# archinetai/audio-diffusion-pytorch

Hardware: NVIDIA H100
Metric: audio-seconds/sec (2ch, 2^18 len) VSampler 50-step (higher is better)
Workload: dtype bf16

## Files before the change

audio_diffusion_pytorch_b200/csrc/common.cuh:

```cuda
#pragma once
#include <cuda.h>
#include <cuda_runtime.h>
#include <stdarg.h>
#include <stdint.h>
#include <stdio.h>

#include "../../include/adp_b200.h"

namespace adp {

int set_error(const char* fmt, ...);

#define ADP_CHECK(cond, ...)                         \
  do {                                               \
    if (!(cond)) return ::adp::set_error(__VA_ARGS__); \
  } while (0)

#define ADP_CUDA(expr)                                                                   \
  do {                                                                                   \
    cudaError_t e_ = (expr);                                                             \
    if (e_ != cudaSuccess)                                                               \
      return ::adp::set_error("%s failed: %s (%s:%d)", #expr, cudaGetErrorString(e_),    \
                              __FILE__, __LINE__);                                       \
  } while (0)

#define ADP_LAUNCH_CHECK() ADP_CUDA(cudaGetLastError())

int make_tmap_bf16(CUtensorMap* out, const void* base, int rank, const uint64_t* dims,
                   const uint64_t* strides_bytes, const uint32_t* box, int swizzle_bytes);

inline cudaStream_t as_stream(adp_stream_t s) { return reinterpret_cast<cudaStream_t>(s); }

struct SmemAttrCache { size_t set[64] = {}; };
template <typename Kern>
inline cudaError_t ensure_dyn_smem(Kern kernel, size_t bytes, SmemAttrCache& cache) {
  int dev = 0;
  cudaError_t e = cudaGetDevice(&dev);
  if (e != cudaSuccess) return e;
  size_t& cur = cache.set[dev & 63];
  if (bytes <= cur) return cudaSuccess;
  e = cudaFuncSetAttribute((const void*)kernel, cudaFuncAttributeMaxDynamicSharedMemorySize, (int)bytes);
  if (e == cudaSuccess) cur = bytes;
  return e;
}

extern int g_pdl;
template <typename Kern, typename... Args>
inline cudaError_t launch_k(Kern kernel, dim3 grid, dim3 block, size_t smem, cudaStream_t st,
                            Args... args) {
  cudaLaunchConfig_t cfg = {};
  cfg.gridDim = grid;
  cfg.blockDim = block;
  cfg.dynamicSmemBytes = smem;
  cfg.stream = st;
  cudaLaunchAttribute attr[1];
  attr[0].id = cudaLaunchAttributeProgrammaticStreamSerialization;
  attr[0].val.programmaticStreamSerializationAllowed = g_pdl ? 1 : 0;
  cfg.attrs = attr;
  cfg.numAttrs = 1;
  void* ptrs[] = {(void*)&args...};
  return cudaLaunchKernelExC(&cfg, (const void*)kernel, ptrs);
}

int num_sms();

template <typename K>
inline int one_wave_gx(K kernel, int threads, size_t smem, int B, int n_tiles) {
  int occ = 1;
  if (cudaOccupancyMaxActiveBlocksPerMultiprocessor(&occ, kernel, threads, smem) != cudaSuccess || occ < 1)
    occ = 1;
  int gx = (occ * num_sms()) / B;
  if (gx < 1) gx = 1;
  if (gx > n_tiles) gx = n_tiles;
  return gx;
}

inline int blocks_per_batch(int n_tiles, int B, int z = 1) {
  int gx = (num_sms() * 4 + B * z - 1) / (B * z);
  if (gx > n_tiles) gx = n_tiles;
  return gx < 1 ? 1 : gx;
}

inline bool ln_row_layout(int C, int* lpr, int* vpl) {
  const int vpr = C / 8;
  if (vpr <= 32) {
    int p = 1;
    while (p < vpr) p <<= 1;
    *lpr = p; *vpl = 1;
  } else {
    *lpr = 32; *vpl = (vpr + 31) / 32;
  }
  return *lpr * *vpl != vpr;
}

inline int capped_grid(int64_t n, int threads) {
  int64_t g = (n + threads - 1) / threads;
  if (g < 1) g = 1;
  if (g > num_sms() * 16) g = num_sms() * 16;
  return static_cast<int>(g);
}

}
```

audio_diffusion_pytorch_b200/csrc/conv_gemm.cu:

```cuda
#include "common.cuh"
#include "ptx.cuh"

namespace adp {

int g_debug[8] = {0, 0, 0, 0, 0, 0, 0, 0};

constexpr int kMaxStages = 8;
constexpr int kMaxGroups = 8;
constexpr int kSmemPerSM = 228 * 1024;
constexpr int kSmemPerBlock = 227 * 1024;

struct Gemm2Params {
  __nv_bfloat16* out;
  const __nv_bfloat16* residual;
  const float* bias;
  const float* gate;
  double* stats;
  int B, T, tiles_per_batch, c_in, ldo;
  int n_pad, n_valid;
  int ntaps, tap_off0, up_factor;
  int groups, group_size, group_shift;
  int out_fp32, ld_gate;
  int n_tiles_n, total_tiles, tiles_per_cta;
  int a_rows;
// ... 11 lines not shown

struct TileInfo {
  int b, t0, n0, phase, ch0, ntaps, min_off;
};

template <int BM>
__device__ __forceinline__ TileInfo tile_info(const Gemm2Params& p, int tile, int BN) {
  TileInfo ti;
  const int m_tile = tile / p.n_tiles_n;
  const int n_tile = tile - m_tile * p.n_tiles_n;
  ti.b = m_tile / p.tiles_per_batch;
  ti.t0 = (m_tile - ti.b * p.tiles_per_batch) * BM;
  ti.n0 = n_tile * BN;
  ti.phase = ti.n0 / p.n_pad;
  ti.ch0 = ti.n0 - ti.phase * p.n_pad;
  if (p.up_factor > 1) {
    if (ti.phase == 0) { ti.ntaps = 2; ti.min_off = -1; }
    else if (ti.phase == p.up_factor - 1) { ti.ntaps = 2; ti.min_off = 0; }
    else { ti.ntaps = 1; ti.min_off = 0; }
  } else {
    ti.ntaps = p.ntaps;
    ti.min_off = p.tap_off0;
  }
  return ti;
}

__device__ __forceinline__ float silu_tanh(float z) {
  float t;
  asm("tanh.approx.f32 %0, %1;" : "=f"(t) : "f"(0.5f * z));
  const float hz = 0.5f * z;
  return fmaf(hz, t, hz);
}

struct WarpStats {
  int cur_g = -1;
  float s = 0.f, q = 0.f;
  template <int NW>
  __device__ __forceinline__ void flush(float (*slots)[NW], int w, int lane) {
    const float ws = warp_sum(s), wq = warp_sum(q);
    if (lane == 0 && cur_g >= 0) { slots[2 * cur_g][w] += ws; slots[2 * cur_g + 1][w] += wq; }
    s = 0.f; q = 0.f;
  }
  template <int NW>
  __device__ __forceinline__ void add(float v, int g, float (*slots)[NW], int w, int lane) {
    if (g != cur_g) { flush(slots, w, lane); cur_g = g; }
    s += v; q += v * v;
  }
};

struct NarrowStats {
  int ch0 = -1;
  float s[4] = {0.f, 0.f, 0.f, 0.f}, q[4] = {0.f, 0.f, 0.f, 0.f};
  __device__ __forceinline__ void add(int k, float v) { s[k] += v; q[k] += v * v; }
  template <int NW>
  __device__ __forceinline__ void flush(float (*slots)[NW], int w, int lane, int shift, int groups) {
    if (ch0 >= 0) {
#pragma unroll
      for (int k = 0; k < 4; ++k) {
        float a = s[k], b = q[k];
#pragma unroll
        for (int o = 4; o < 32; o <<= 1) {
          a += __shfl_xor_sync(0xffffffffu, a, o);
          b += __shfl_xor_sync(0xffffffffu, b, o);
        }
        if (shift == 2) {
          a += __shfl_xor_sync(0xffffffffu, a, 1);
          b += __shfl_xor_sync(0xffffffffu, b, 1);
        }
        const int col = shift == 0 ? ch0 + 2 * lane + k : ch0 + 8 * k + 2 * (lane & 3);
        const int g = col >> shift;
        if (lane < 4 && (shift != 2 || !(lane & 1)) && (shift != 0 || k < 2) && g < groups) {
          slots[2 * g][w] += a;
          slots[2 * g + 1][w] += b;
        }
        s[k] = 0.f; q[k] = 0.f;
      }
    }
    ch0 = -1;
  }
};

template <int BM> constexpr int gemm_threads() { return 2 * BM + 32; }

template <int BM, int BN, int SW, bool XF, bool NARROW>
__global__ void __launch_bounds__(gemm_threads<BM>(), BM == 256 ? 1 : (BN <= 32 ? 3 : (BN <= 64 ? 2 : 1)))
conv_gemm2_kernel(const __grid_constant__ CUtensorMap tmA, const __grid_constant__ CUtensorMap tmW,
                  const Gemm2Params p) {
  static_assert(!NARROW || (BN <= 64 && !XF), "narrow statistics registers: BN <= 64 without XF");
  static_assert(BM == 128 || (BM == 256 && BN == 64 && !XF && !NARROW),
                "256-row tiles: BN = 64, without the A transform or the narrow statistics");
  constexpr int BK = SW / 2;
  constexpr int NACC = BN / 2;
  constexpr int kConsumers = 2 * BM;
  constexpr int kConsumerWarps = BM / 16;
  constexpr uint32_t kWTapBytes = BN * SW;
  extern __shared__ uint8_t smem_raw[];
  __shared__ uint64_t full_bar[kMaxStages], empty_bar[kMaxStages];
  __shared__ float s_part[2 * kMaxGroups][kConsumerWarps];
  __shared__ __align__(16) float s_coef[XF ? 2 * 1024 : 4];

  pdl_launch_dependents();
  const int warp = warp_id_uniform();
  const int lane = threadIdx.x & 31;
  const uint32_t raw = smem_u32(smem_raw);
  uint8_t* ring = smem_raw + ((1024u - (raw & 1023u)) & 1023u);

  const int tile_begin = blockIdx.x * p.tiles_per_cta;
  int tile_end = tile_begin + p.tiles_per_cta;
  if (tile_end > p.total_tiles) tile_end = p.total_tiles;

  if (threadIdx.x < 2 * kMaxGroups * kConsumerWarps) (&s_part[0][0])[threadIdx.x] = 0.f;
  if (warp == kConsumerWarps && lane == 0) {
    for (int s = 0; s < p.n_stages; ++s) { mbar_init(&full_bar[s], 1); mbar_init(&empty_bar[s], kConsumerWarps); }
    fence_mbar_init();
    tma_prefetch_desc(&tmA);
    tma_prefetch_desc(&tmW);
  }
  __syncthreads();
  if (warp == kConsumerWarps) {
    const uint32_t a_bytes = static_cast<uint32_t>(BM / 128) * p.a_rows * SW;
    const int total_it = (tile_end - tile_begin) * p.k_stages;
    int early = 0;
    if (p.early_w) {
      early = total_it < p.n_stages ? total_it : p.n_stages;
      if (elect_one()) {
        int tile = tile_begin, ks = 0;
        for (int it = 0; it < early; ++it) {
          const TileInfo ti = tile_info<BM>(p, tile, BN);
          uint8_t* st = ring + it * p.stage_bytes;
          mbar_arrive_expect_tx(&full_bar[it], static_cast<uint32_t>(p.kc) * (a_bytes + ti.ntaps * kWTapBytes));
          for (int c = 0; c < p.kc; ++c) {
            const int k0 = (ks * p.kc + c) * BK;
            uint8_t* wdst = st + p.kc * p.a_sub_bytes + c * p.max_taps * p.w_sub_bytes;
            for (int tap = 0; tap < ti.ntaps; ++tap)
              tma_load_2d(wdst + tap * p.w_sub_bytes, &tmW, &full_bar[it], tap * p.c_in + k0, ti.n0);
          }
          if (++ks == p.k_stages) { ks = 0; ++tile; }
        }
      }
      __syncwarp();
    }
    pdl_wait();
    int s = 0, it = 0;
    uint32_t ph = 0;
    for (int tile = tile_begin; tile < tile_end; ++tile) {
      const TileInfo ti = tile_info<BM>(p, tile, BN);
      const uint32_t tx = static_cast<uint32_t>(p.kc) * (a_bytes + ti.ntaps * kWTapBytes);
      for (int ks = 0; ks < p.k_stages; ++ks, ++it) {
        const bool armed = it < early;
        if (!armed) mbar_wait(&empty_bar[s], ph ^ 1);
        uint8_t* st = ring + s * p.stage_bytes;
        if (elect_one()) {
          if (!armed) mbar_arrive_expect_tx(&full_bar[s], tx);
          for (int c = 0; c < p.kc; ++c) {
            const int k0 = (ks * p.kc + c) * BK;
            tma_load_3d(st + c * p.a_sub_bytes, &tmA, &full_bar[s], k0, ti.t0 + ti.min_off, ti.b);
            if constexpr (BM == 256)
              tma_load_3d(st + c * p.a_sub_bytes + 128 * SW, &tmA, &full_bar[s], k0, ti.t0 + ti.min_off + 128, ti.b);
            if (armed) continue;
            uint8_t* wdst = st + p.kc * p.a_sub_bytes + c * p.max_taps * p.w_sub_bytes;
            for (int tap = 0; tap < ti.ntaps; ++tap)
              tma_load_2d(wdst + tap * p.w_sub_bytes, &tmW, &full_bar[s], tap * p.c_in + k0, ti.n0);
          }
        }
        __syncwarp();
        if (++s == p.n_stages) { s = 0; ph ^= 1; }
      }
    }
    return;
  }

  pdl_wait();
  const int tid = threadIdx.x;
  const int wg = tid >> 7;
  const int r0 = wg * 64 + (warp & 3) * 16 + (lane >> 2);
  const int cq = 2 * (lane & 3);
  const bool do_stats = p.stats != nullptr;
  const bool narrow = NARROW && p.group_shift >= 0 && p.group_shift < 3;
  WarpStats acc_st;
  NarrowStats nar_st;
  int cur_b = -1, coef_b = -1;

  auto publish_stats = [&](int b_done) {
    acc_st.flush(s_part, warp, lane);
    acc_st.cur_g = -1;
    if (narrow) nar_st.flush(s_part, warp, lane, p.group_shift, p.groups);
    named_bar_sync(1, kConsumers);
    if (tid < 2 * p.groups) {
      float tot = 0.f;
#pragma unroll
      for (int w = 0; w < kConsumerWarps; ++w) { tot += s_part[tid][w]; s_part[tid][w] = 0.f; }
      if (tot != 0.f) atomicAdd(p.stats + static_cast<size_t>(b_done) * 2 * p.groups + tid, static_cast<double>(tot));
    }
    named_bar_sync(1, kConsumers);
  };

  const uint64_t desc0 = gmma_desc_kmajor<SW>(smem_u32(ring));
  const uint32_t stage_u = static_cast<uint32_t>(p.stage_bytes) >> 4;
  const uint32_t a_sub_u = static_cast<uint32_t>(p.a_sub_bytes) >> 4;
  const uint32_t w_sub_u = static_cast<uint32_t>(p.w_sub_bytes) >> 4;
  const uint32_t w_base_u = static_cast<uint32_t>(p.kc) * a_sub_u;
  const uint32_t wg_row_u = static_cast<uint32_t>(wg * 64 * SW) >> 4;
  int s = 0;
  uint32_t ph = 0;
  for (int tile = tile_begin; tile < tile_end; ++tile) {
    const TileInfo ti = tile_info<BM>(p, tile, BN);
    if constexpr (XF) {
      if (ti.b != coef_b) {
        named_bar_sync(1, kConsumers);
        const int gsz = p.c_in / p.gn_groups;
        const double inv_n = 1.0 / (static_cast<double>(gsz) * p.T);
        for (int ch = tid; ch < p.c_in; ch += kConsumers) {
          const int g = ch / gsz;
          const double mean = p.gn_stats[(static_cast<size_t>(ti.b) * p.gn_groups + g) * 2] * inv_n;
          const float var = fmaxf(static_cast<float>(
              p.gn_stats[(static_cast<size_t>(ti.b) * p.gn_groups + g) * 2 + 1] * inv_n - mean * mean), 0.f);
          const float ga = __ldg(p.gn_gamma + ch) * rsqrtf(var + p.gn_eps);
          s_coef[2 * ch] = ga;
          s_coef[2 * ch + 1] = __ldg(p.gn_beta + ch) - static_cast<float>(mean) * ga;
        }
        named_bar_sync(1, kConsumers);
        coef_b = ti.b;
      }
    }
    float acc[NACC];
    uint32_t accumulate = 0;
    int prev_s = -1;
    for (int ks = 0; ks < p.k_stages; ++ks) {
      mbar_wait(&full_bar[s], ph);
      if constexpr (XF) {
        constexpr int CPR = SW / 16;
        constexpr int CPT = CPR / 2 > 0 ? CPR / 2 : 1;
        uint8_t* st = ring + s * p.stage_bytes;
        for (int c = 0; c < p.kc; ++c) {
          uint8_t* sub = st + c * p.a_sub_bytes;
          const float* cf = s_coef + (ks * p.kc + c) * BK * 2;
          for (int rr = tid >> 1; rr < p.a_rows; rr += kConsumers / 2) {
            const int t = ti.t0 + ti.min_off + rr;
            if (t < 0 || t >= p.T) continue;
            const uint32_t row_off = static_cast<uint32_t>(rr) * SW;
            const int swz = (row_off >> 7) & (CPR - 1);
#pragma unroll
            for (int q = 0; q < CPT; ++q) {
              const int pc = (CPR >= 2) ? (tid & 1) * CPT + q : 0;
              if (CPR < 2 && (tid & 1)) continue;
              const int lc = pc ^ swz;
              uint4* ptr = reinterpret_cast<uint4*>(sub + row_off + pc * 16);
              const uint4 u = *ptr;
              const float4* c4 = reinterpret_cast<const float4*>(cf + lc * 16);
              const float4 k0 = c4[0], k1 = c4[1], k2 = c4[2], k3 = c4[3];
              const float2 f0 = unpack_bf16(u.x), f1 = unpack_bf16(u.y);
              const float2 f2 = unpack_bf16(u.z), f3 = unpack_bf16(u.w);
              uint4 o;
              o.x = pack_bf16(silu_tanh(f0.x * k0.x + k0.y), silu_tanh(f0.y * k0.z + k0.w));
              o.y = pack_bf16(silu_tanh(f1.x * k1.x + k1.y), silu_tanh(f1.y * k1.z + k1.w));
              o.z = pack_bf16(silu_tanh(f2.x * k2.x + k2.y), silu_tanh(f2.y * k2.z + k2.w));
              o.w = pack_bf16(silu_tanh(f3.x * k3.x + k3.y), silu_tanh(f3.y * k3.z + k3.w));
              *ptr = o;
            }
          }
        }
        fence_proxy_async_smem();
        named_bar_sync(1, kConsumers);
      }
      wgmma_fence();
      const uint64_t sdesc = desc0 + static_cast<uint64_t>(s * stage_u);
      for (int c = 0; c < p.kc; ++c) {
        const uint64_t adesc = sdesc + c * a_sub_u + wg_row_u;
        const uint64_t wdesc = sdesc + w_base_u + c * p.max_taps * w_sub_u;
        for (int tap = 0; tap < ti.ntaps; ++tap) {
#pragma unroll
          for (int kk = 0; kk < BK / 16; ++kk) {
            Wgmma<BN>::template ss<0, 0>(acc, adesc + ((tap * SW + kk * 32) >> 4),
                                         wdesc + tap * w_sub_u + ((kk * 32) >> 4), accumulate);
            accumulate = 1;
          }
        }
      }
      wgmma_commit();
      wgmma_wait<1>();
      if (prev_s >= 0) {
        __syncwarp();
        if (lane == 0) mbar_arrive(&empty_bar[prev_s]);
      }
      prev_s = s;
      if (++s == p.n_stages) { s = 0; ph ^= 1; }
    }
    wgmma_wait<0>();
    acc_fence(acc);
    __syncwarp();
    if (lane == 0) mbar_arrive(&empty_bar[prev_s]);

    if (do_stats && ti.b != cur_b) {
      if (cur_b >= 0) publish_stats(cur_b);
      cur_b = ti.b;
    }
    if (narrow && ti.ch0 != nar_st.ch0) {
      nar_st.flush(s_part, warp, lane, p.group_shift, p.groups);
      nar_st.ch0 = ti.ch0;
    }
    const int t_lo = ti.t0 + r0, t_hi = t_lo + 8;
    const bool ok_lo = t_lo < p.T, ok_hi = t_hi < p.T;
    const size_t col_off = static_cast<size_t>(ti.phase) * p.n_valid;
    const size_t off_lo = (static_cast<size_t>(ti.b) * p.T + (ok_lo ? t_lo : 0)) * p.ldo + col_off;
    const size_t off_hi = (static_cast<size_t>(ti.b) * p.T + (ok_hi ? t_hi : 0)) * p.ldo + col_off;
    const float* gate_row = p.gate ? p.gate + static_cast<size_t>(ti.b) * p.ld_gate : nullptr;
#pragma unroll
    for (int jb = 0; jb < BN / 8; ++jb) {
      if (ti.ch0 + jb * 8 >= p.n_valid) break;
      const int ch = ti.ch0 + jb * 8 + cq;
      const float2 bb = p.bias ? make_float2(__ldg(p.bias + ch), __ldg(p.bias + ch + 1)) : make_float2(0.f, 0.f);
      const float2 gg = gate_row ? make_float2(__ldg(gate_row + ch), __ldg(gate_row + ch + 1)) : make_float2(1.f, 1.f);
      float v[4];
      v[0] = (acc[4 * jb + 0] + bb.x) * gg.x; v[1] = (acc[4 * jb + 1] + bb.y) * gg.y;
      v[2] = (acc[4 * jb + 2] + bb.x) * gg.x; v[3] = (acc[4 * jb + 3] + bb.y) * gg.y;
      if (p.out_fp32) {
        float* o = reinterpret_cast<float*>(p.out);
        if (ok_lo) *reinterpret_cast<float2*>(o + off_lo + ch) = make_float2(v[0], v[1]);
        if (ok_hi) *reinterpret_cast<float2*>(o + off_hi + ch) = make_float2(v[2], v[3]);
        continue;
      }
      if (p.residual) {
        if (ok_lo) {
          const float2 r = unpack_bf16(__ldg(reinterpret_cast<const unsigned int*>(p.residual + off_lo + ch)));
          v[0] += r.x; v[1] += r.y;
        }
        if (ok_hi) {
          const float2 r = unpack_bf16(__ldg(reinterpret_cast<const unsigned int*>(p.residual + off_hi + ch)));
          v[2] += r.x; v[3] += r.y;
        }
      }
      const uint32_t o_lo = pack_bf16(v[0], v[1]), o_hi = pack_bf16(v[2], v[3]);
      if (ok_lo) *reinterpret_cast<uint32_t*>(p.out + off_lo + ch) = o_lo;
      if (ok_hi) *reinterpret_cast<uint32_t*>(p.out + off_hi + ch) = o_hi;
      if (do_stats) {
        const float2 q_lo = ok_lo ? unpack_bf16(o_lo) : make_float2(0.f, 0.f);
        const float2 q_hi = ok_hi ? unpack_bf16(o_hi) : make_float2(0.f, 0.f);
        if (p.group_shift >= 3) {
          const int g = (ti.ch0 + jb * 8) >> p.group_shift;
          acc_st.add(q_lo.x, g, s_part, warp, lane); acc_st.add(q_lo.y, g, s_part, warp, lane);
          acc_st.add(q_hi.x, g, s_part, warp, lane); acc_st.add(q_hi.y, g, s_part, warp, lane);
        } else if (narrow) {
          if (p.group_shift == 0) {
            nar_st.add(0, q_lo.x); nar_st.add(0, q_hi.x);
            nar_st.add(1, q_lo.y); nar_st.add(1, q_hi.y);
          } else if (jb < 4) {
            nar_st.add(jb, q_lo.x); nar_st.add(jb, q_lo.y);
            nar_st.add(jb, q_hi.x); nar_st.add(jb, q_hi.y);
          }
        } else {
          float cs[2] = {q_lo.x + q_hi.x, q_lo.y + q_hi.y};
          float cs2[2] = {q_lo.x * q_lo.x + q_hi.x * q_hi.x, q_lo.y * q_lo.y + q_hi.y * q_hi.y};
#pragma unroll
          for (int e = 0; e < 2; ++e)
#pragma unroll
            for (int o = 4; o < 32; o <<= 1) {
              cs[e] += __shfl_xor_sync(0xffffffffu, cs[e], o);
              cs2[e] += __shfl_xor_sync(0xffffffffu, cs2[e], o);
            }
#pragma unroll
          for (int i = 0; i < 8; ++i) {
            const float v = __shfl_sync(0xffffffffu, cs[i & 1], i >> 1);
            const float v2 = __shfl_sync(0xffffffffu, cs2[i & 1], i >> 1);
            const int g = (ti.ch0 + jb * 8 + i) / p.group_size;
            if (lane == 0) { s_part[2 * g][warp] += v; s_part[2 * g + 1][warp] += v2; }
          }
        }
      }
    }
  }
  if (do_stats && cur_b >= 0) publish_stats(cur_b);
}

template <int BM, int BN, int SW, bool XF, bool NARROW>
static int launch_gemm2(const adp_conv_gemm_args& a, cudaStream_t stream) {
  constexpr int BK = SW / 2;
  constexpr int kThreads = gemm_threads<BM>();
  auto kernel = conv_gemm2_kernel<BM, BN, SW, XF, NARROW>;
  const int tiles_per_batch = (a.T + BM - 1) / BM;
  const bool up = a.up_factor > 1;
  const int max_taps = up ? 2 : a.ntaps;
  const int span = up ? 1 : a.ntaps - 1;
  const int a_rows = 128 + span;
  const int k_chunks = a.c_in / BK;

  Gemm2Params p;
  p.a_sub_bytes = ((BM + span) * SW + 1023) / 1024 * 1024;
  p.w_sub_bytes = (BN * SW + 1023) / 1024 * 1024;
  p.max_taps = max_taps;
  const int chunk_bytes = p.a_sub_bytes + max_taps * p.w_sub_bytes;

  const int w_iters = k_chunks * max_taps;
  int occ = 1;
  if (BM == 256) occ = 1;
  else if (BN <= 64 && w_iters <= 8) occ = 3;
  else if (BN <= 128 && w_iters <= 12) occ = 2;
  if (XF && occ > (BN <= 64 ? 2 : 1)) occ = BN <= 64 ? 2 : 1;
  if (g_debug[3] > 0) occ = g_debug[3];
  static int static_smem = -1;
  if (static_smem < 0) {
    cudaFuncAttributes fa;
    ADP_CUDA(cudaFuncGetAttributes(&fa, kernel));
    static_smem = static_cast<int>(fa.sharedSizeBytes);
  }
  auto budget_of = [&](int o) {
    int per_cta = kSmemPerSM / o - 1024;
    if (per_cta > kSmemPerBlock) per_cta = kSmemPerBlock;
    return per_cta - static_smem - 1024;
  };
  while (occ > 1 && budget_of(occ) < 2 * chunk_bytes) --occ;
  const int budget = budget_of(occ);
  int kc = 1;
  while (kc * 2 <= 4 && k_chunks % (kc * 2) == 0 && kc * max_taps * (BK / 16) < 8 &&
         2 * (kc * 2) * chunk_bytes <= budget)
    kc *= 2;
  if (g_debug[5] > 0 && k_chunks % g_debug[5] == 0) kc = g_debug[5];
  p.kc = kc;
  p.k_stages = k_chunks / kc;
  p.stage_bytes = kc * chunk_bytes;
  int n_stages = budget / p.stage_bytes;
  if (n_stages > kMaxStages) n_stages = kMaxStages;
  if (n_stages < 2)
    return set_error("adp_conv_gemm: stage of %d bytes does not fit (BN=%d)", p.stage_bytes, BN);
  p.n_stages = n_stages;
  const size_t smem = static_cast<size_t>(n_stages) * p.stage_bytes + 1024;

  CUtensorMap tmA, tmW;
  {
    const uint64_t dims[3] = {(uint64_t)a.c_in, (uint64_t)a.T, (uint64_t)a.B};
    const uint64_t strides[2] = {(uint64_t)a.lda * 2, (uint64_t)a.T * a.lda * 2};
    const uint32_t box[3] = {(uint32_t)BK, (uint32_t)a_rows, 1};
    if (int e = make_tmap_bf16(&tmA, a.a, 3, dims, strides, box, SW)) return e;
  }
  {
    const uint64_t dims[2] = {(uint64_t)a.k_total, (uint64_t)a.phases * a.n_pad};
    const uint64_t strides[1] = {(uint64_t)a.k_total * 2};
    const uint32_t box[2] = {(uint32_t)BK, (uint32_t)BN};
    if (int e = make_tmap_bf16(&tmW, a.w, 2, dims, strides, box, SW)) return e;
  }

  static SmemAttrCache smem_cache;
  ADP_CUDA(ensure_dyn_smem(kernel, smem, smem_cache));
  int occ_hw = 1;
  if (cudaOccupancyMaxActiveBlocksPerMultiprocessor(&occ_hw, kernel, kThreads, smem) != cudaSuccess ||
      occ_hw < 1)
    occ_hw = 1;
  if (occ > occ_hw) occ = occ_hw;

  p.out = static_cast<__nv_bfloat16*>(a.out);
  p.residual = static_cast<const __nv_bfloat16*>(a.residual);
  p.bias = a.bias;
  p.gate = a.gate;
  p.stats = a.stats;
  p.B = a.B;
  p.T = a.T;
  p.tiles_per_batch = tiles_per_batch;
  p.c_in = a.c_in;
  p.ldo = a.ldo;
  p.n_pad = a.n_pad;
  p.n_valid = a.n_valid;
  p.ntaps = a.ntaps;
  p.tap_off0 = a.tap_off[0];
  p.up_factor = a.up_factor;
  p.groups = a.stats ? a.groups : 0;
  p.group_size = a.stats ? a.n_valid / a.groups : 1;
  p.group_shift = -1;
  for (int sft = 0; sft < 16; ++sft)
    if ((1 << sft) == p.group_size) p.group_shift = sft;
  p.out_fp32 = a.out_fp32;
  p.ld_gate = a.ld_gate > 0 ? a.ld_gate : a.n_valid;
  p.n_tiles_n = a.phases * a.n_pad / BN;
  p.total_tiles = a.B * tiles_per_batch * p.n_tiles_n;
  p.a_rows = a_rows;
  p.early_w = g_debug[2];
  p.gn_stats = a.gn_stats;
  p.gn_gamma = a.gn_gamma;
  p.gn_beta = a.gn_beta;
  p.gn_eps = a.gn_eps;
  p.gn_groups = a.gn_groups > 0 ? a.gn_groups : 1;

  const int slots = occ * num_sms();
  int grid = p.total_tiles < slots ? p.total_tiles : slots;
  p.tiles_per_cta = (p.total_tiles + grid - 1) / grid;
  grid = (p.total_tiles + p.tiles_per_cta - 1) / p.tiles_per_cta;
  ADP_CUDA(launch_k(kernel, dim3(grid), dim3(kThreads), smem, stream, tmA, tmW, p));
  ADP_LAUNCH_CHECK();
  return 0;
}

static bool needs_narrow(const adp_conv_gemm_args& a) {
  const int group_size = a.stats ? a.n_valid / a.groups : 0;
  return group_size == 1 || group_size == 2 || group_size == 4 || g_debug[7] != 0;
}

template <int SW>
static int dispatch_bn2(const adp_conv_gemm_args& a, int bn, cudaStream_t s) {
  if (a.gn_stats) {
    switch (bn) {
      case 16: return launch_gemm2<128, 16, SW, true, false>(a, s);
      case 32: return launch_gemm2<128, 32, SW, true, false>(a, s);
      case 64: return launch_gemm2<128, 64, SW, true, false>(a, s);
      case 128: return launch_gemm2<128, 128, SW, true, false>(a, s);
      case 256: return launch_gemm2<128, 256, SW, true, false>(a, s);
    }
  }
  const bool narrow = needs_narrow(a);
  switch (bn) {
    case 16: return narrow ? launch_gemm2<128, 16, SW, false, true>(a, s) : launch_gemm2<128, 16, SW, false, false>(a, s);
    case 32: return narrow ? launch_gemm2<128, 32, SW, false, true>(a, s) : launch_gemm2<128, 32, SW, false, false>(a, s);
    case 64: return narrow ? launch_gemm2<128, 64, SW, false, true>(a, s) : launch_gemm2<128, 64, SW, false, false>(a, s);
    case 128: return launch_gemm2<128, 128, SW, false, false>(a, s);
    case 256: return launch_gemm2<128, 256, SW, false, false>(a, s);
  }
  return set_error("adp_conv_gemm: unsupported N tile %d", bn);
}

static bool has_256_rows(const adp_conv_gemm_args& a) {
  return a.n_pad % 64 == 0 && a.c_in % 64 == 0 && !a.gn_stats && !needs_narrow(a) && a.T >= 256;
}

}

namespace adp { extern int g_mid_threads; }

extern "C" int adp_debug_set(int key, int value) {
  if (key == 8) {
    if (value != 128 && value != 256) return adp::set_error("adp_debug_set: key 8 takes 128 or 256");
    adp::g_mid_threads = value;
    return 0;
  }
  if (key < 0 || key >= 8) return adp::set_error("adp_debug_set: bad key %d", key);
  if (key == 4 && value != 0 && value != 128 && value != 256)
    return adp::set_error("adp_debug_set: key 4 takes 0, 128 or 256");
  adp::g_debug[key] = value;
  if (key == 6) adp::g_pdl = value;
  return 0;
}

extern "C" int adp_conv_gemm(const adp_conv_gemm_args* args, adp_stream_t stream) {
  using namespace adp;
  ADP_CHECK(args != nullptr, "adp_conv_gemm: null args");
  const adp_conv_gemm_args& a = *args;
  ADP_CHECK(a.a && a.w && a.out, "adp_conv_gemm: null a/w/out");
  ADP_CHECK(a.B > 0 && a.T > 0, "adp_conv_gemm: bad B=%d T=%d", a.B, a.T);
  ADP_CHECK(a.c_in >= 16 && a.c_in % 16 == 0, "adp_conv_gemm: c_in=%d must be a multiple of 16",
            a.c_in);
  ADP_CHECK(a.lda % 8 == 0 && a.ldo % 8 == 0 && a.k_total % 8 == 0 && a.lda >= a.c_in,
            "adp_conv_gemm: pitches lda=%d ldo=%d k_total=%d must be multiples of 8", a.lda, a.ldo,
            a.k_total);
  ADP_CHECK(a.n_valid > 0 && a.n_valid % 8 == 0 && a.n_valid <= a.n_pad && a.n_pad % 16 == 0,
            "adp_conv_gemm: n_valid=%d n_pad=%d", a.n_valid, a.n_pad);
  ADP_CHECK(a.phases >= 1, "adp_conv_gemm: phases=%d", a.phases);
  ADP_CHECK(a.ld_gate % 4 == 0, "adp_conv_gemm: ld_gate=%d must be a multiple of 4", a.ld_gate);
  if (a.up_factor > 1) {
    ADP_CHECK(a.phases == a.up_factor, "adp_conv_gemm: phases (%d) != up_factor (%d)", a.phases,
              a.up_factor);
    ADP_CHECK(a.k_total >= 2 * a.c_in, "adp_conv_gemm: upsample weights need 2 tap slots");
  } else {
    ADP_CHECK(a.ntaps >= 1 && a.ntaps <= 3 && a.phases == 1, "adp_conv_gemm: ntaps=%d phases=%d",
              a.ntaps, a.phases);
    ADP_CHECK(a.k_total >= a.ntaps * a.c_in, "adp_conv_gemm: k_total too small");
    for (int i = 1; i < a.ntaps; ++i)
      ADP_CHECK(a.tap_off[i] == a.tap_off[i - 1] + 1,
                "adp_conv_gemm: tap offsets must be consecutive and ascending");
  }
  if (a.out_fp32) {
    ADP_CHECK(!a.residual && !a.stats, "adp_conv_gemm: out_fp32 excludes residual/stats");
  }
  if (a.gn_stats) {
    ADP_CHECK(a.c_in <= 1024, "adp_conv_gemm: fused GroupNorm supports c_in <= 1024");
    ADP_CHECK(a.gn_gamma && a.gn_beta && a.gn_groups > 0 && a.c_in % a.gn_groups == 0 && a.lda == a.c_in,
              "adp_conv_gemm: fused GroupNorm needs gamma/beta, groups | c_in and a dense input");
  }
  if (a.stats) {
    ADP_CHECK(a.groups > 0 && a.groups <= kMaxGroups && a.n_valid % a.groups == 0,
              "adp_conv_gemm: groups=%d n_valid=%d (fused statistics handle <= %d groups)",
              a.groups, a.n_valid, kMaxGroups);
  }
  int bn = a.block_n;
  if (bn == 0) {
    const long m_tiles = (long)a.B * ((a.T + 127) / 128);
    const int k_per_tile = (a.up_factor > 1 ? 2 : a.ntaps) * a.c_in;
    const int widest = !a.gn_stats && k_per_tile <= 1024 ? 64 : 128;
    bn = 16;
    for (int cand = widest; cand >= 16; cand >>= 1) {
      if (a.n_pad % cand) continue;
      const long tiles = m_tiles * (a.phases * a.n_pad / cand);
      if (tiles >= 96 || cand <= 64) { bn = cand; break; }
    }
  }
  bool rows256 = false;
  if (g_debug[4] == 256) {
    ADP_CHECK(has_256_rows(a) && (a.block_n == 0 || a.block_n == 64),
              "adp_conv_gemm: no 256-row tile for block_n=%d c_in=%d T=%d", a.block_n, a.c_in, a.T);
    rows256 = true;
  } else if (a.block_n == 0 && g_debug[4] != 128) {
    rows256 = bn == 128 && has_256_rows(a);
  }
  ADP_CHECK(a.n_pad % bn == 0, "adp_conv_gemm: N tile %d does not divide n_pad %d", bn, a.n_pad);
  cudaStream_t s = as_stream(stream);
  if (rows256) return launch_gemm2<256, 64, 128, false, false>(a, s);
  if (a.c_in % 64 == 0) return dispatch_bn2<128>(a, bn, s);
  if (a.c_in % 32 == 0) return dispatch_bn2<64>(a, bn, s);
  return dispatch_bn2<32>(a, bn, s);
}
```

audio_diffusion_pytorch_b200/csrc/ptx.cuh:

```cuda
#pragma once
#include <cuda.h>
#include <cuda_bf16.h>
#include <cuda_runtime.h>
#include <stdint.h>

namespace adp {

__device__ __forceinline__ uint32_t smem_u32(const void* p) {
  return static_cast<uint32_t>(__cvta_generic_to_shared(p));
}

__device__ __forceinline__ int warp_id_uniform() {
  return __shfl_sync(0xffffffffu, static_cast<int>(threadIdx.x >> 5), 0);
}
__device__ __forceinline__ bool elect_one() {
  uint32_t pred;
  asm volatile(
      "{\n\t.reg .pred p;\n\t"
      "elect.sync _|p, 0xffffffff;\n\t"
      "selp.u32 %0, 1, 0, p;\n\t}"
      : "=r"(pred));
  return pred != 0;
}

__device__ __forceinline__ void mbar_init(uint64_t* bar, uint32_t count) {
  asm volatile("mbarrier.init.shared::cta.b64 [%0], %1;" ::"r"(smem_u32(bar)), "r"(count));
}
__device__ __forceinline__ void fence_mbar_init() {
  asm volatile("fence.mbarrier_init.release.cluster;" ::: "memory");
}
__device__ __forceinline__ void fence_proxy_async_smem() {
  asm volatile("fence.proxy.async.shared::cta;" ::: "memory");
}
__device__ __forceinline__ void mbar_arrive_expect_tx(uint64_t* bar, uint32_t bytes) {
  asm volatile("mbarrier.arrive.expect_tx.shared::cta.b64 _, [%0], %1;" ::"r"(smem_u32(bar)),
               "r"(bytes)
               : "memory");
}
__device__ __forceinline__ void mbar_arrive(uint64_t* bar) {
  asm volatile("mbarrier.arrive.shared::cta.b64 _, [%0];" ::"r"(smem_u32(bar)) : "memory");
}
__device__ __forceinline__ bool mbar_try_wait(uint64_t* bar, uint32_t parity) {
  uint32_t ok;
  asm volatile(
      "{\n\t.reg .pred p;\n\t"
      "mbarrier.try_wait.parity.shared::cta.b64 p, [%1], %2;\n\t"
      "selp.u32 %0, 1, 0, p;\n\t}"
      : "=r"(ok)
      : "r"(smem_u32(bar)), "r"(parity)
      : "memory");
  return ok != 0;
}
static __device__ __noinline__ void mbar_wait_slow(uint64_t* bar, uint32_t parity) {
  uint32_t spins = 0;
  while (!mbar_try_wait(bar, parity)) {
    if (++spins > (1u << 24)) __trap();
  }
}
__device__ __forceinline__ void mbar_wait(uint64_t* bar, uint32_t parity) {
  if (mbar_try_wait(bar, parity)) return;
  mbar_wait_slow(bar, parity);
}

__device__ __forceinline__ void tma_prefetch_desc(const CUtensorMap* m) {
  asm volatile("prefetch.tensormap [%0];" ::"l"(reinterpret_cast<uint64_t>(m)) : "memory");
}
__device__ __forceinline__ void tma_load_2d(void* smem_dst, const CUtensorMap* m, uint64_t* bar,
                                            int c0, int c1) {
  asm volatile(
      "cp.async.bulk.tensor.2d.shared::cluster.global.mbarrier::complete_tx::bytes"
      " [%0], [%1, {%3, %4}], [%2];" ::"r"(smem_u32(smem_dst)),
      "l"(reinterpret_cast<uint64_t>(m)), "r"(smem_u32(bar)), "r"(c0), "r"(c1)
      : "memory");
}
__device__ __forceinline__ void tma_load_3d(void* smem_dst, const CUtensorMap* m, uint64_t* bar,
                                            int c0, int c1, int c2) {
  asm volatile(
      "cp.async.bulk.tensor.3d.shared::cluster.global.mbarrier::complete_tx::bytes"
      " [%0], [%1, {%3, %4, %5}], [%2];" ::"r"(smem_u32(smem_dst)),
      "l"(reinterpret_cast<uint64_t>(m)), "r"(smem_u32(bar)), "r"(c0), "r"(c1), "r"(c2)
      : "memory");
}
__device__ __forceinline__ void tma_load_4d(void* smem_dst, const CUtensorMap* m, uint64_t* bar,
                                            int c0, int c1, int c2, int c3) {
  asm volatile(
      "cp.async.bulk.tensor.4d.shared::cluster.global.mbarrier::complete_tx::bytes"
      " [%0], [%1, {%3, %4, %5, %6}], [%2];" ::"r"(smem_u32(smem_dst)),
      "l"(reinterpret_cast<uint64_t>(m)), "r"(smem_u32(bar)), "r"(c0), "r"(c1), "r"(c2), "r"(c3)
      : "memory");
}

__device__ __forceinline__ void wgmma_fence() {
  asm volatile("wgmma.fence.sync.aligned;" ::: "memory");
}
__device__ __forceinline__ void wgmma_commit() {
  asm volatile("wgmma.commit_group.sync.aligned;" ::: "memory");
}
template <int N>
__device__ __forceinline__ void wgmma_wait() {
  asm volatile("wgmma.wait_group.sync.aligned %0;" ::"n"(N) : "memory");
}
template <int R>
__device__ __forceinline__ void acc_fence(float (&d)[R]) {
#pragma unroll
  for (int i = 0; i < R; ++i) asm volatile("" : "+f"(d[i])::"memory");
}

template <int N> struct Wgmma;
template <> struct Wgmma<16> {
  template <int TA, int TB>
  static __device__ __forceinline__ void ss(float (&d)[8], uint64_t a, uint64_t b, uint32_t acc) {
    asm volatile(
        "{\n\t.reg .pred p;\n\tsetp.ne.b32 p, %10, 0;\n\t"
        "wgmma.mma_async.sync.aligned.m64n16k16.f32.bf16.bf16 {%0, %1, %2, %3, %4, %5, %6, %7}, %8, %9, p, 1, 1, %11, %12;\n\t}"
        : "+f"(d[0]), "+f"(d[1]), "+f"(d[2]), "+f"(d[3]), "+f"(d[4]), "+f"(d[5]), "+f"(d[6]), "+f"(d[7])
        : "l"(a), "l"(b), "r"(acc), "n"(TA), "n"(TB));
  }
};
template <> struct Wgmma<32> {
  template <int TA, int TB>
  static __device__ __forceinline__ void ss(float (&d)[16], uint64_t a, uint64_t b, uint32_t acc) {
    asm volatile(
        "{\n\t.reg .pred p;\n\tsetp.ne.b32 p, %18, 0;\n\t"
        "wgmma.mma_async.sync.aligned.m64n32k16.f32.bf16.bf16 {%0, %1, %2, %3, %4, %5, %6, %7, %8, %9, %10, %11, %12, %13, %14, %15}, %16, %17, p, 1, 1, %19, %20;\n\t}"
        : "+f"(d[0]), "+f"(d[1]), "+f"(d[2]), "+f"(d[3]), "+f"(d[4]), "+f"(d[5]), "+f"(d[6]), "+f"(d[7]), "+f"(d[8]), "+f"(d[9]), "+f"(d[10]), "+f"(d[11]), "+f"(d[12]), "+f"(d[13]), "+f"(d[14]), "+f"(d[15])
        : "l"(a), "l"(b), "r"(acc), "n"(TA), "n"(TB));
  }
  template <int TB>
  static __device__ __forceinline__ void rs(float (&d)[16], const uint32_t (&a)[4], uint64_t b, uint32_t acc) {
    asm volatile(
        "{\n\t.reg .pred p;\n\tsetp.ne.b32 p, %21, 0;\n\t"
        "wgmma.mma_async.sync.aligned.m64n32k16.f32.bf16.bf16 {%0, %1, %2, %3, %4, %5, %6, %7, %8, %9, %10, %11, %12, %13, %14, %15}, {%16, %17, %18, %19}, %20, p, 1, 1, %22;\n\t}"
        : "+f"(d[0]), "+f"(d[1]), "+f"(d[2]), "+f"(d[3]), "+f"(d[4]), "+f"(d[5]), "+f"(d[6]), "+f"(d[7]), "+f"(d[8]), "+f"(d[9]), "+f"(d[10]), "+f"(d[11]), "+f"(d[12]), "+f"(d[13]), "+f"(d[14]), "+f"(d[15])
        : "r"(a[0]), "r"(a[1]), "r"(a[2]), "r"(a[3]), "l"(b), "r"(acc), "n"(TB));
  }
};
template <> struct Wgmma<64> {
  template <int TA, int TB>
  static __device__ __forceinline__ void ss(float (&d)[32], uint64_t a, uint64_t b, uint32_t acc) {
    asm volatile(
        "{\n\t.reg .pred p;\n\tsetp.ne.b32 p, %34, 0;\n\t"
        "wgmma.mma_async.sync.aligned.m64n64k16.f32.bf16.bf16 {%0, %1, %2, %3, %4, %5, %6, %7, %8, %9, %10, %11, %12, %13, %14, %15, %16, %17, %18, %19, %20, %21, %22, %23, %24, %25, %26, %27, %28, %29, %30, %31}, %32, %33, p, 1, 1, %35, %36;\n\t}"
        : "+f"(d[0]), "+f"(d[1]), "+f"(d[2]), "+f"(d[3]), "+f"(d[4]), "+f"(d[5]), "+f"(d[6]), "+f"(d[7]), "+f"(d[8]), "+f"(d[9]), "+f"(d[10]), "+f"(d[11]), "+f"(d[12]), "+f"(d[13]), "+f"(d[14]), "+f"(d[15]), "+f"(d[16]), "+f"(d[17]), "+f"(d[18]), "+f"(d[19]), "+f"(d[20]), "+f"(d[21]), "+f"(d[22]), "+f"(d[23]), "+f"(d[24]), "+f"(d[25]), "+f"(d[26]), "+f"(d[27]), "+f"(d[28]), "+f"(d[29]), "+f"(d[30]), "+f"(d[31])
        : "l"(a), "l"(b), "r"(acc), "n"(TA), "n"(TB));
  }
  template <int TB>
  static __device__ __forceinline__ void rs(float (&d)[32], const uint32_t (&a)[4], uint64_t b, uint32_t acc) {
    asm volatile(
        "{\n\t.reg .pred p;\n\tsetp.ne.b32 p, %37, 0;\n\t"
        "wgmma.mma_async.sync.aligned.m64n64k16.f32.bf16.bf16 {%0, %1, %2, %3, %4, %5, %6, %7, %8, %9, %10, %11, %12, %13, %14, %15, %16, %17, %18, %19, %20, %21, %22, %23, %24, %25, %26, %27, %28, %29, %30, %31}, {%32, %33, %34, %35}, %36, p, 1, 1, %38;\n\t}"
        : "+f"(d[0]), "+f"(d[1]), "+f"(d[2]), "+f"(d[3]), "+f"(d[4]), "+f"(d[5]), "+f"(d[6]), "+f"(d[7]), "+f"(d[8]), "+f"(d[9]), "+f"(d[10]), "+f"(d[11]), "+f"(d[12]), "+f"(d[13]), "+f"(d[14]), "+f"(d[15]), "+f"(d[16]), "+f"(d[17]), "+f"(d[18]), "+f"(d[19]), "+f"(d[20]), "+f"(d[21]), "+f"(d[22]), "+f"(d[23]), "+f"(d[24]), "+f"(d[25]), "+f"(d[26]), "+f"(d[27]), "+f"(d[28]), "+f"(d[29]), "+f"(d[30]), "+f"(d[31])
        : "r"(a[0]), "r"(a[1]), "r"(a[2]), "r"(a[3]), "l"(b), "r"(acc), "n"(TB));
  }
};
template <> struct Wgmma<128> {
  template <int TA, int TB>
  static __device__ __forceinline__ void ss(float (&d)[64], uint64_t a, uint64_t b, uint32_t acc) {
    asm volatile(
        "{\n\t.reg .pred p;\n\tsetp.ne.b32 p, %66, 0;\n\t"
        "wgmma.mma_async.sync.aligned.m64n128k16.f32.bf16.bf16 {%0, %1, %2, %3, %4, %5, %6, %7, %8, %9, %10, %11, %12, %13, %14, %15, %16, %17, %18, %19, %20, %21, %22, %23, %24, %25, %26, %27, %28, %29, %30, %31, %32, %33, %34, %35, %36, %37, %38, %39, %40, %41, %42, %43, %44, %45, %46, %47, %48, %49, %50, %51, %52, %53, %54, %55, %56, %57, %58, %59, %60, %61, %62, %63}, %64, %65, p, 1, 1, %67, %68;\n\t}"
        : "+f"(d[0]), "+f"(d[1]), "+f"(d[2]), "+f"(d[3]), "+f"(d[4]), "+f"(d[5]), "+f"(d[6]), "+f"(d[7]), "+f"(d[8]), "+f"(d[9]), "+f"(d[10]), "+f"(d[11]), "+f"(d[12]), "+f"(d[13]), "+f"(d[14]), "+f"(d[15]), "+f"(d[16]), "+f"(d[17]), "+f"(d[18]), "+f"(d[19]), "+f"(d[20]), "+f"(d[21]), "+f"(d[22]), "+f"(d[23]), "+f"(d[24]), "+f"(d[25]), "+f"(d[26]), "+f"(d[27]), "+f"(d[28]), "+f"(d[29]), "+f"(d[30]), "+f"(d[31]), "+f"(d[32]), "+f"(d[33]), "+f"(d[34]), "+f"(d[35]), "+f"(d[36]), "+f"(d[37]), "+f"(d[38]), "+f"(d[39]), "+f"(d[40]), "+f"(d[41]), "+f"(d[42]), "+f"(d[43]), "+f"(d[44]), "+f"(d[45]), "+f"(d[46]), "+f"(d[47]), "+f"(d[48]), "+f"(d[49]), "+f"(d[50]), "+f"(d[51]), "+f"(d[52]), "+f"(d[53]), "+f"(d[54]), "+f"(d[55]), "+f"(d[56]), "+f"(d[57]), "+f"(d[58]), "+f"(d[59]), "+f"(d[60]), "+f"(d[61]), "+f"(d[62]), "+f"(d[63])
        : "l"(a), "l"(b), "r"(acc), "n"(TA), "n"(TB));
  }
// ... 125 lines not shown
```

Before: 171.2.

## Add CTA-pair cluster path multicasting A tiles across paired GEMM blocks

Adds an optional 2-CTA cluster mode for the conv GEMM, in which paired CTAs handle adjacent N tiles. Each CTA loads half of the shared A operand and multicasts it to both through TMA, and the empty barriers count consumers from both CTAs. The goal is to halve global/L2 traffic for activations. It also clamps occupancy to the number of tiles per SM and routes wide-K upsampling convs to 256-row tiles. The pair path is gated behind a debug flag and adds cluster synchronisation costs.

```diff
diff --git a/audio_diffusion_pytorch_b200/csrc/common.cuh b/audio_diffusion_pytorch_b200/csrc/common.cuh
--- a/audio_diffusion_pytorch_b200/csrc/common.cuh
+++ b/audio_diffusion_pytorch_b200/csrc/common.cuh
@@ -46,20 +46,29 @@
 
 extern int g_pdl;
 template <typename Kern, typename... Args>
-inline cudaError_t launch_k(Kern kernel, dim3 grid, dim3 block, size_t smem, cudaStream_t st,
-                            Args... args) {
+inline cudaError_t launch_kc(Kern kernel, dim3 grid, dim3 block, size_t smem, cudaStream_t st,
+                             int cluster, Args... args) {
   cudaLaunchConfig_t cfg = {};
   cfg.gridDim = grid;
   cfg.blockDim = block;
   cfg.dynamicSmemBytes = smem;
   cfg.stream = st;
-  cudaLaunchAttribute attr[1];
+  cudaLaunchAttribute attr[2];
   attr[0].id = cudaLaunchAttributeProgrammaticStreamSerialization;
   attr[0].val.programmaticStreamSerializationAllowed = g_pdl ? 1 : 0;
+  attr[1].id = cudaLaunchAttributeClusterDimension;
+  attr[1].val.clusterDim.x = cluster;
+  attr[1].val.clusterDim.y = 1;
+  attr[1].val.clusterDim.z = 1;
   cfg.attrs = attr;
-  cfg.numAttrs = 1;
+  cfg.numAttrs = cluster > 1 ? 2 : 1;
   void* ptrs[] = {(void*)&args...};
   return cudaLaunchKernelExC(&cfg, (const void*)kernel, ptrs);
+}
+template <typename Kern, typename... Args>
+inline cudaError_t launch_k(Kern kernel, dim3 grid, dim3 block, size_t smem, cudaStream_t st,
+                            Args... args) {
+  return launch_kc(kernel, grid, block, smem, st, 1, args...);
 }
 
 int num_sms();
diff --git a/audio_diffusion_pytorch_b200/csrc/conv_gemm.cu b/audio_diffusion_pytorch_b200/csrc/conv_gemm.cu
--- a/audio_diffusion_pytorch_b200/csrc/conv_gemm.cu
+++ b/audio_diffusion_pytorch_b200/csrc/conv_gemm.cu
@@ -117,13 +117,15 @@
 
 template <int BM> constexpr int gemm_threads() { return 2 * BM + 32; }
 
-template <int BM, int BN, int SW, bool XF, bool NARROW>
+template <int BM, int BN, int SW, bool XF, bool NARROW, bool PAIR = false>
 __global__ void __launch_bounds__(gemm_threads<BM>(), BM == 256 ? 1 : (BN <= 32 ? 3 : (BN <= 64 ? 2 : 1)))
 conv_gemm2_kernel(const __grid_constant__ CUtensorMap tmA, const __grid_constant__ CUtensorMap tmW,
                   const Gemm2Params p) {
   static_assert(!NARROW || (BN <= 64 && !XF), "narrow statistics registers: BN <= 64 without XF");
   static_assert(BM == 128 || (BM == 256 && BN == 64 && !XF && !NARROW),
                 "256-row tiles: BN = 64, without the A transform or the narrow statistics");
+  static_assert(!PAIR || (BN == 64 && SW == 128 && !XF && !NARROW),
+                "CTA pairs: BN = 64, 64-channel chunks, without the A transform or the narrow statistics");
   constexpr int BK = SW / 2;
   constexpr int NACC = BN / 2;
   constexpr int kConsumers = 2 * BM;
@@ -140,21 +142,33 @@
   const uint32_t raw = smem_u32(smem_raw);
   uint8_t* ring = smem_raw + ((1024u - (raw & 1023u)) & 1023u);
 
-  const int tile_begin = blockIdx.x * p.tiles_per_cta;
-  int tile_end = tile_begin + p.tiles_per_cta;
-  if (tile_end > p.total_tiles) tile_end = p.total_tiles;
+  constexpr int kPair = PAIR ? 2 : 1;
+  int rank = 0, tile_begin, tile_end;
+  if constexpr (PAIR) {
+    rank = static_cast<int>(cluster_ctarank());
+    const int unit_begin = (blockIdx.x >> 1) * p.tiles_per_cta;
+    int unit_end = unit_begin + p.tiles_per_cta;
+    if (unit_end > p.total_tiles / 2) unit_end = p.total_tiles / 2;
+    tile_begin = 2 * unit_begin + rank;
+    tile_end = 2 * unit_end;
+  } else {
+    tile_begin = blockIdx.x * p.tiles_per_cta;
+    tile_end = tile_begin + p.tiles_per_cta;
+    if (tile_end > p.total_tiles) tile_end = p.total_tiles;
+  }
 
   if (threadIdx.x < 2 * kMaxGroups * kConsumerWarps) (&s_part[0][0])[threadIdx.x] = 0.f;
   if (warp == kConsumerWarps && lane == 0) {
-    for (int s = 0; s < p.n_stages; ++s) { mbar_init(&full_bar[s], 1); mbar_init(&empty_bar[s], kConsumerWarps); }
+    for (int s = 0; s < p.n_stages; ++s) { mbar_init(&full_bar[s], 1); mbar_init(&empty_bar[s], kPair * kConsumerWarps); }
     fence_mbar_init();
     tma_prefetch_desc(&tmA);
     tma_prefetch_desc(&tmW);
   }
-  __syncthreads();
+  if constexpr (PAIR) cluster_sync();
+  else __syncthreads();
   if (warp == kConsumerWarps) {
     const uint32_t a_bytes = static_cast<uint32_t>(BM / 128) * p.a_rows * SW;
-    const int total_it = (tile_end - tile_begin) * p.k_stages;
+    const int total_it = (PAIR ? (tile_end - tile_begin + 1) / 2 : tile_end - tile_begin) * p.k_stages;
     int early = 0;
     if (p.early_w) {
       early = total_it < p.n_stages ? total_it : p.n_stages;
@@ -170,7 +184,7 @@
             for (int tap = 0; tap < ti.ntaps; ++tap)
               tma_load_2d(wdst + tap * p.w_sub_bytes, &tmW, &full_bar[it], tap * p.c_in + k0, ti.n0);
           }
-          if (++ks == p.k_stages) { ks = 0; ++tile; }
+          if (++ks == p.k_stages) { ks = 0; tile += kPair; }
         }
       }
       __syncwarp();
@@ -178,7 +192,7 @@
     pdl_wait();
     int s = 0, it = 0;
     uint32_t ph = 0;
-    for (int tile = tile_begin; tile < tile_end; ++tile) {
+    for (int tile = tile_begin; tile < tile_end; tile += kPair) {
       const TileInfo ti = tile_info<BM>(p, tile, BN);
       const uint32_t tx = static_cast<uint32_t>(p.kc) * (a_bytes + ti.ntaps * kWTapBytes);
       for (int ks = 0; ks < p.k_stages; ++ks, ++it) {
@@ -189,9 +203,17 @@
           if (!armed) mbar_arrive_expect_tx(&full_bar[s], tx);
           for (int c = 0; c < p.kc; ++c) {
             const int k0 = (ks * p.kc + c) * BK;
-            tma_load_3d(st + c * p.a_sub_bytes, &tmA, &full_bar[s], k0, ti.t0 + ti.min_off, ti.b);
-            if constexpr (BM == 256)
-              tma_load_3d(st + c * p.a_sub_bytes + 128 * SW, &tmA, &full_bar[s], k0, ti.t0 + ti.min_off + 128, ti.b);
+            if constexpr (PAIR) {
+              const int j0 = (p.kc * (BM / 128) == 1 ? it : c * (BM / 128));
+              for (int h = 0; h < BM / 128; ++h)
+                if (((j0 + h) & 1) == rank)
+                  tma_load_3d_multicast(st + c * p.a_sub_bytes + h * 128 * SW, &tmA, &full_bar[s], k0,
+                                        ti.t0 + ti.min_off + h * 128, ti.b, 0x3);
+            } else {
+              tma_load_3d(st + c * p.a_sub_bytes, &tmA, &full_bar[s], k0, ti.t0 + ti.min_off, ti.b);
+              if constexpr (BM == 256)
+                tma_load_3d(st + c * p.a_sub_bytes + 128 * SW, &tmA, &full_bar[s], k0, ti.t0 + ti.min_off + 128, ti.b);
+            }
             if (armed) continue;
             uint8_t* wdst = st + p.kc * p.a_sub_bytes + c * p.max_taps * p.w_sub_bytes;
             for (int tap = 0; tap < ti.ntaps; ++tap)
@@ -202,6 +224,7 @@
         if (++s == p.n_stages) { s = 0; ph ^= 1; }
       }
     }
+    if constexpr (PAIR) cluster_sync();
     return;
   }
 
@@ -236,9 +259,10 @@
   const uint32_t w_sub_u = static_cast<uint32_t>(p.w_sub_bytes) >> 4;
   const uint32_t w_base_u = static_cast<uint32_t>(p.kc) * a_sub_u;
   const uint32_t wg_row_u = static_cast<uint32_t>(wg * 64 * SW) >> 4;
+  const uint32_t peer_empty = PAIR ? mapa_shared(smem_u32(&empty_bar[0]), rank ^ 1) : 0u;
   int s = 0;
   uint32_t ph = 0;
-  for (int tile = tile_begin; tile < tile_end; ++tile) {
+  for (int tile = tile_begin; tile < tile_end; tile += kPair) {
     const TileInfo ti = tile_info<BM>(p, tile, BN);
     if constexpr (XF) {
       if (ti.b != coef_b) {
@@ -316,7 +340,10 @@
       wgmma_wait<1>();
       if (prev_s >= 0) {
         __syncwarp();
-        if (lane == 0) mbar_arrive(&empty_bar[prev_s]);
+        if (lane == 0) {
+          mbar_arrive(&empty_bar[prev_s]);
+          if constexpr (PAIR) mbar_arrive_cluster(peer_empty + 8u * prev_s);
+        }
       }
       prev_s = s;
       if (++s == p.n_stages) { s = 0; ph ^= 1; }
@@ -324,7 +351,10 @@
     wgmma_wait<0>();
     acc_fence(acc);
     __syncwarp();
-    if (lane == 0) mbar_arrive(&empty_bar[prev_s]);
+    if (lane == 0) {
+      mbar_arrive(&empty_bar[prev_s]);
+      if constexpr (PAIR) mbar_arrive_cluster(peer_empty + 8u * prev_s);
+    }
 
     if (do_stats && ti.b != cur_b) {
       if (cur_b >= 0) publish_stats(cur_b);
@@ -405,13 +435,15 @@
     }
   }
   if (do_stats && cur_b >= 0) publish_stats(cur_b);
-}
-
-template <int BM, int BN, int SW, bool XF, bool NARROW>
+  if constexpr (PAIR) cluster_sync();
+}
+
+template <int BM, int BN, int SW, bool XF, bool NARROW, bool PAIR = false>
 static int launch_gemm2(const adp_conv_gemm_args& a, cudaStream_t stream) {
   constexpr int BK = SW / 2;
   constexpr int kThreads = gemm_threads<BM>();
-  auto kernel = conv_gemm2_kernel<BM, BN, SW, XF, NARROW>;
+  constexpr int kPair = PAIR ? 2 : 1;
+  auto kernel = conv_gemm2_kernel<BM, BN, SW, XF, NARROW, PAIR>;
   const int tiles_per_batch = (a.T + BM - 1) / BM;
   const bool up = a.up_factor > 1;
   const int max_taps = up ? 2 : a.ntaps;
@@ -431,6 +463,12 @@
   else if (BN <= 64 && w_iters <= 8) occ = 3;
   else if (BN <= 128 && w_iters <= 12) occ = 2;
   if (XF && occ > (BN <= 64 ? 2 : 1)) occ = BN <= 64 ? 2 : 1;
+  if (BM == 128) {
+    const long tiles = (long)a.B * tiles_per_batch * (a.phases * a.n_pad / BN);
+    const long per_sm = (tiles + num_sms() - 1) / num_sms();
+    if (occ > per_sm) occ = static_cast<int>(per_sm);
+    else if (occ == 1 && per_sm == 2) occ = 2;
+  }
   if (g_debug[3] > 0) occ = g_debug[3];
   static int static_smem = -1;
   if (static_smem < 0) {
@@ -514,11 +552,38 @@
   p.gn_eps = a.gn_eps;
   p.gn_groups = a.gn_groups > 0 ? a.gn_groups : 1;
 
-  const int slots = occ * num_sms();
-  int grid = p.total_tiles < slots ? p.total_tiles : slots;
-  p.tiles_per_cta = (p.total_tiles + grid - 1) / grid;
-  grid = (p.total_tiles + p.tiles_per_cta - 1) / p.tiles_per_cta;
-  ADP_CUDA(launch_k(kernel, dim3(grid), dim3(kThreads), smem, stream, tmA, tmW, p));
+  int slots = occ * num_sms() / kPair;
+  if constexpr (PAIR) {
+    static int cluster_cache[64][2] = {};
+    int dev = 0;
+    ADP_CUDA(cudaGetDevice(&dev));
+    int* cached = cluster_cache[dev & 63];
+    if (cached[0] != static_cast<int>(smem)) {
+      cudaLaunchConfig_t cfg = {};
+      cfg.gridDim = dim3(kPair);
+      cfg.blockDim = dim3(kThreads);
+      cfg.dynamicSmemBytes = smem;
+      cudaLaunchAttribute attr;
+      attr.id = cudaLaunchAttributeClusterDimension;
+      attr.val.clusterDim.x = kPair;
+      attr.val.clusterDim.y = 1;
+      attr.val.clusterDim.z = 1;
+      cfg.attrs = &attr;
+      cfg.numAttrs = 1;
+      int clusters = 0;
+      ADP_CUDA(cudaOccupancyMaxActiveClusters(&clusters, (const void*)kernel, &cfg));
+      cached[0] = static_cast<int>(smem);
+      cached[1] = clusters;
+    }
+    ADP_CHECK(cached[1] >= 1, "adp_conv_gemm: a CTA pair with %zu bytes of shared memory each cannot be resident",
+              smem);
+    if (slots > cached[1]) slots = cached[1];
+  }
+  const int units = p.total_tiles / kPair;
+  int grid = units < slots ? units : slots;
+  p.tiles_per_cta = (units + grid - 1) / grid;
+  grid = (units + p.tiles_per_cta - 1) / p.tiles_per_cta;
+  ADP_CUDA(launch_kc(kernel, dim3(grid * kPair), dim3(kThreads), smem, stream, kPair, tmA, tmW, p));
   ADP_LAUNCH_CHECK();
   return 0;
 }
@@ -526,6 +591,15 @@
 static bool needs_narrow(const adp_conv_gemm_args& a) {
   const int group_size = a.stats ? a.n_valid / a.groups : 0;
   return group_size == 1 || group_size == 2 || group_size == 4 || g_debug[7] != 0;
+}
+
+static bool has_pairs(const adp_conv_gemm_args& a, int bn) {
+  return bn == 64 && a.c_in % 64 == 0 && !a.gn_stats && !needs_narrow(a) && a.up_factor <= 1 &&
+         a.phases == 1 && (a.n_pad / bn) % 2 == 0;
+}
+
+static bool use_pairs(const adp_conv_gemm_args& a, int bn) {
+  return g_debug[0] == 1 && has_pairs(a, bn);
 }
 
 template <int SW>
@@ -543,7 +617,11 @@
   switch (bn) {
     case 16: return narrow ? launch_gemm2<128, 16, SW, false, true>(a, s) : launch_gemm2<128, 16, SW, false, false>(a, s);
     case 32: return narrow ? launch_gemm2<128, 32, SW, false, true>(a, s) : launch_gemm2<128, 32, SW, false, false>(a, s);
-    case 64: return narrow ? launch_gemm2<128, 64, SW, false, true>(a, s) : launch_gemm2<128, 64, SW, false, false>(a, s);
+    case 64:
+      if (narrow) return launch_gemm2<128, 64, SW, false, true>(a, s);
+      if constexpr (SW == 128)
+        if (use_pairs(a, bn)) return launch_gemm2<128, 64, SW, false, false, true>(a, s);
+      return launch_gemm2<128, 64, SW, false, false>(a, s);
     case 128: return launch_gemm2<128, 128, SW, false, false>(a, s);
     case 256: return launch_gemm2<128, 256, SW, false, false>(a, s);
   }
@@ -630,11 +708,14 @@
               "adp_conv_gemm: no 256-row tile for block_n=%d c_in=%d T=%d", a.block_n, a.c_in, a.T);
     rows256 = true;
   } else if (a.block_n == 0 && g_debug[4] != 128) {
-    rows256 = bn == 128 && has_256_rows(a);
+    const bool up_wide_k = a.up_factor > 1 && bn == 64 && 2 * (a.c_in / 64) > 12;
+    rows256 = (bn == 128 || up_wide_k) && has_256_rows(a);
   }
   ADP_CHECK(a.n_pad % bn == 0, "adp_conv_gemm: N tile %d does not divide n_pad %d", bn, a.n_pad);
   cudaStream_t s = as_stream(stream);
-  if (rows256) return launch_gemm2<256, 64, 128, false, false>(a, s);
+  if (rows256)
+    return use_pairs(a, 64) ? launch_gemm2<256, 64, 128, false, false, true>(a, s)
+                                 : launch_gemm2<256, 64, 128, false, false>(a, s);
   if (a.c_in % 64 == 0) return dispatch_bn2<128>(a, bn, s);
   if (a.c_in % 32 == 0) return dispatch_bn2<64>(a, bn, s);
   return dispatch_bn2<32>(a, bn, s);
diff --git a/audio_diffusion_pytorch_b200/csrc/ptx.cuh b/audio_diffusion_pytorch_b200/csrc/ptx.cuh
--- a/audio_diffusion_pytorch_b200/csrc/ptx.cuh
+++ b/audio_diffusion_pytorch_b200/csrc/ptx.cuh
@@ -62,6 +62,23 @@
   mbar_wait_slow(bar, parity);
 }
 
+__device__ __forceinline__ uint32_t cluster_ctarank() {
+  uint32_t r;
+  asm volatile("mov.u32 %0, %%cluster_ctarank;" : "=r"(r));
+  return r;
+}
+__device__ __forceinline__ void cluster_sync() {
+  asm volatile("barrier.cluster.arrive.release.aligned;\n\tbarrier.cluster.wait.acquire.aligned;" ::: "memory");
+}
+__device__ __forceinline__ uint32_t mapa_shared(uint32_t smem_addr, uint32_t rank) {
+  uint32_t r;
+  asm volatile("mapa.shared::cluster.u32 %0, %1, %2;" : "=r"(r) : "r"(smem_addr), "r"(rank));
+  return r;
+}
+__device__ __forceinline__ void mbar_arrive_cluster(uint32_t cluster_addr) {
+  asm volatile("mbarrier.arrive.release.cluster.shared::cluster.b64 _, [%0];" ::"r"(cluster_addr) : "memory");
+}
+
 __device__ __forceinline__ void tma_prefetch_desc(const CUtensorMap* m) {
   asm volatile("prefetch.tensormap [%0];" ::"l"(reinterpret_cast<uint64_t>(m)) : "memory");
 }
@@ -79,6 +96,14 @@
       "cp.async.bulk.tensor.3d.shared::cluster.global.mbarrier::complete_tx::bytes"
       " [%0], [%1, {%3, %4, %5}], [%2];" ::"r"(smem_u32(smem_dst)),
       "l"(reinterpret_cast<uint64_t>(m)), "r"(smem_u32(bar)), "r"(c0), "r"(c1), "r"(c2)
+      : "memory");
+}
+__device__ __forceinline__ void tma_load_3d_multicast(void* smem_dst, const CUtensorMap* m, uint64_t* bar,
+                                                      int c0, int c1, int c2, uint16_t cta_mask) {
+  asm volatile(
+      "cp.async.bulk.tensor.3d.shared::cluster.global.mbarrier::complete_tx::bytes.multicast::cluster"
+      " [%0], [%1, {%3, %4, %5}], [%2], %6;" ::"r"(smem_u32(smem_dst)),
+      "l"(reinterpret_cast<uint64_t>(m)), "r"(smem_u32(bar)), "r"(c0), "r"(c1), "r"(c2), "h"(cta_mask)
       : "memory");
 }
 __device__ __forceinline__ void tma_load_4d(void* smem_dst, const CUtensorMap* m, uint64_t* bar,
```

After: 173.2 (median of 6 runs). 1.2% higher.
